# surftemp/cae_tools

Hardware: AMD Instinct MI355X
Metric: train images/sec (16x16->256x256, batch 64) (higher is better)
Workload: dtype f32

## Files before the change

cae_tools_amd/csrc/engine_choose.h:

```cpp
#pragma once

namespace {


#define S2_SHAPES(X) X(2, 1) X(4, 2) X(8, 4) X(6, 3)
#define S2_KERNELS(X, CI, CO) X(CI, CO, 3, 3) X(CI, CO, 4, 4) X(CI, CO, 3, 4) X(CI, CO, 4, 3)

template <int CI, int CO, int KH, int KW>
struct S2Shape { static constexpr int cin = CI, cout = CO, kh = KH, kw = KW; };

template <class F>
auto s2_for_shape(const ConvLayer& L, F fn) {
#define ONE(CI, CO, KH_, KW_) \
    if (L.cin == CI && L.cout == CO && L.kh == KH_ && L.kw == KW_) return fn(S2Shape<CI, CO, KH_, KW_>{});
#define PAIR(CI, CO) S2_KERNELS(ONE, CI, CO)
    S2_SHAPES(PAIR)
#undef PAIR
#undef ONE
    return false;
}

bool s2_shape_ok(const ConvLayer& L) { return L.transposed && L.stride == 2 && s2_for_shape(L, [](auto) { return true; }); }

bool s2_eligible(const cae_engine* e, const ConvLayer& L) { return e->use_s2 && L.sh_w >= 0 && s2_shape_ok(L); }
// ... 308 lines not shown
        if (h.n_seg + 1 > kHeadMaxSeg) return no("segments");
        h.o_bias[i] = take(cnt);
        h.seg[h.n_seg++] = HeadSeg{e->params + e->fc[i].b_off, i == 3 ? std::min(cnt, e->fc[3].nout) : cnt, h.o_bias[i], i == 3 ? 1 : 0};
    }
    for (int i = 0; i < 4; i++) {
        if (e->fc[i].nin % 4) return no("nin4");
        const int tiles = i == 3 ? h.tiles_per_wg : (e->fc[i].nout + 15) / 16;
        h.fc_split[i] = stage_split(tiles, e->fc[i].nin);
    }
    lds_bytes = (size_t)align_up(top, 4) * sizeof(float);
    return lds_bytes <= 152 * 1024 || no("lds");
}


bool tail_plan(const cae_engine* e, const StepArgs& a, TailArgs& t, size_t& lds_bytes, const char** why = nullptr) {
    auto no = [&](const char* reason) {
        if (why) *why = reason;
        return false;
    };
    if (!e->use_s2) return no("mode");
    if (a.syncing()) return no("syncing");
    if (e->variational) return no("variational");
    memset(&t, 0, sizeof t);
    const ConvLayer& P = e->enc.back();
    double* acc = e->gradacc();
    t.B = a.batch;
    for (int i = 0; i < 3; i++) {
        const FcLayer& F = e->fc[i];
        if (F.nin % 4 || F.nout % 4) return no("fc4");
        if (16 * F.nout / 4 > 2 * kHeadThreads) return no("panel");
        HeadFc& f = t.fc[i];
        f.nin = F.nin; f.nout = F.nout; f.relu = F.relu ? 1 : 0;
        f.w = e->params + F.w_off; f.bias = e->params + F.b_off;
        f.act = e->fptr(F.act_off); f.grad = e->fptr(F.grad_off);
        f.w_acc = acc + F.w_off; f.b_acc = acc + F.b_off;
        t.w4[i] = F.nin * F.nout / 4;
        if (t.w4[i] > 2 * kHeadThreads) return no("weights");
        const int r16 = (F.nin + 15) / 16 * 16;
        t.ldw[i] = r16 % 32 == 0 ? r16 + 16 : r16;
    }
    if (P.cout > kHeadMaxC || e->fc[0].nin != P.cout * P.hout * P.wout) return no("channels");
    t.y_last = e->fptr(P.act_off);
    t.g_last = e->fptr(P.grad_off);
    t.gamma = e->params + P.gamma_off;
    t.beta = e->params + P.beta_off;
    t.saved = e->bn_saved(P.bn_index);
    t.stats = e->bn_stats(P.bn_index);
    t.C = P.cout;
    t.hw = P.hout * P.wout;
    auto ld_of = [](int n) { return (n + 31) / 32 * 32 + 4; };
    t.ld2 = ld_of(e->fc[2].nout);
    t.ld1 = ld_of(e->fc[1].nout);
    t.ld0 = ld_of(e->fc[0].nout);
    int64_t top = 0;
    auto take = [&](int64_t floats) { return lds_take(top, floats); };
    t.o_c = take(4 * (int64_t)P.cout);
    t.o_red = take(2 * 2 * (int64_t)kHeadWaves);
    t.o_g2 = take(16 * (int64_t)t.ld2 + 32);
    t.o_g1 = take(16 * (int64_t)t.ld1 + 32);
    t.o_g0 = take(16 * (int64_t)t.ld0 + 32);
    t.o_y = take(16 * (int64_t)e->fc[0].nin + 32);
    t.o_gx = take(16 * (int64_t)e->fc[0].nin + 32);
    top = align_up(top, 4);
    t.zero4 = (int)((top - t.o_g2) / 4);
    int64_t wmax = 0;
    for (int i = 0; i < 3; i++) wmax = std::max<int64_t>(wmax, (int64_t)e->fc[i].nout * t.ldw[i]);
    t.o_w = take(wmax + 64);
    t.o_part = take(kHeadWaves * 256);
    lds_bytes = (size_t)align_up(top, 4) * sizeof(float);
    if (lds_bytes > 152 * 1024) return no("lds");
    for (int i = 0; i < 3; i++) t.sp_d[i] = stage_split((e->fc[2 - i].nin + 15) / 16, e->fc[2 - i].nout);
    for (int i = 0; i < 3; i++) t.sp_w[i] = stage_split(((e->fc[2 - i].nout + 15) / 16) * ((e->fc[2 - i].nin + 16) / 16), 16);
    return true;
}

enum DecFwdK {
    DF_FUSED_LAST,
    DF_ROWS,
    DF_S2,
    DF_CT_LDS,
    DF_IG,
    DF_UP
};
enum DecBwdK {
    DB_FUSED_LAST,
    DB_ROWS,
    DB_S2,
    DB_CT_LDS,
    DB_IG,
    DB_GENERIC
};

int s2_fwd_epi(const cae_engine* e, int l, bool train, bool external_loss) {
    if (l + 1 < (int)e->dec.size()) return train ? S2_RAW_STATS : S2_RAW;
    if (external_loss) return S2_RAW;
    return train ? S2_SIGMSE : S2_SIGOUT;
}

bool rows_ok(const cae_engine* e, const ConvLayer& L, int l) {
    return l + 1 < (int)e->dec.size() && l > 0 && e->dec[l - 1].has_bn && rows_bwd_ok(e, L);
}

DecFwdK choose_dec_fwd(const cae_engine* e, const ConvLayer& L, int l, int B, bool train, bool external_loss) {
    const bool last = l + 1 == (int)e->dec.size();
    if (last && train && !external_loss && last_fused_ok(e, L)) return DF_FUSED_LAST;
    if (rows_ok(e, L, l)) return DF_ROWS;
    if (s2_eligible(e, L)) return DF_S2;
    if (e->use_s2 && !last && L.stride == 2 && L.kh <= 4 && L.kw <= 4) {
        CtFwd c;
        int waves = 0;
        size_t lds = 0;
        return ct_fwd_plan(e, B, L, l, c, waves, lds) ? DF_CT_LDS : DF_IG;
    }
    return DF_UP;
}

DecBwdK choose_dec_bwd(const cae_engine* e, const ConvLayer& L, int l, int B, bool external_loss) {
    const bool last = l + 1 == (int)e->dec.size();
    if (last && !external_loss && last_fused_ok(e, L)) return DB_FUSED_LAST;
    if (rows_ok(e, L, l)) return DB_ROWS;
    if (s2_eligible(e, L)) return DB_S2;
    if (e->use_s2) {
        CtBwdPlan p;
        return ct_bwd_plan(e, B, L, l, p) ? DB_CT_LDS : DB_IG;
    }
    return DB_GENERIC;
}

bool enc_conv0_fits_adam(const cae_engine* e, const StepArgs& a, const ConvLayer& L) {
    return e->use_s2 && !a.syncing() && a.world == 1 && L.cout <= 64 &&
           (int64_t)L.cin * L.cout * L.kh * L.kw <= 4096 && (int64_t)a.batch * L.hout * L.wout < kDivSmallMaxN &&
           L.hout * L.wout < kDivSmallMaxD && L.in_elems() < (1 << 24) && L.out_elems() < (1 << 24) &&
           (int64_t)a.batch * L.in_elems() < (1 << 30) && (int64_t)a.batch * L.out_elems() < (1 << 30) &&
           e->bn_stat_off[L.bn_index] == e->off_zero_begin;
}

bool enc_conv0_in_adam_ok(const cae_engine* e, const StepArgs& a, const ConvLayer& L) {
    return a.adam_follows && e->x_published && enc_conv0_fits_adam(e, a, L);
}

const char* head_staging(const HeadArgs& h) {
    const int per = h.enc[0].cin * h.enc[0].hin * h.enc[0].win;
    if (per & 3) return "scalar";
    return h.B * (per >> 2) <= 4 * kHeadThreads ? "direct" : "gather4";
}

}

extern "C" {

int cae_debug_plan(const cae_engine* e, int batch, int train, char* out, int64_t out_bytes) {
    if (!e || !out || out_bytes < 1) return fail(CAE_ERR_ARG, "cae_debug_plan: bad argument");
    if (batch < 1 || batch > e->max_batch) return fail(CAE_ERR_ARG, "cae_debug_plan: batch %d outside 1 .. %d", batch, e->max_batch);
    const bool tr = train != 0, ext = e->variational;
    const StepArgs a{0, nullptr, batch, batch, batch, tr, true, nullptr, nullptr, false};
    std::string s;
    char line[512];
    bool head_fused = false;
    {
        HeadArgs h;
        size_t lds = 0;
        const char* why = "";
        head_fused = head_plan(e, a, h, lds, &why);
        if (head_fused) {
            int straddle = 0;
            for (int j = 0; j < kHeadW4 && j * kHeadThreads < h.w_total4; j++) straddle += h.piece_m[j] == -1;
            const int T = (e->fc[3].nout + 15) / 16;
            snprintf(line, sizeof line,
                     "head fwd=fused enc=%d grid=%dx%d stage=%s w4=%d late=%d straddle=%d fc0=%d:%d fc1=%d:%d fc2=%d:%d fc3=%d:%d lds=%zu\n",
                     h.n_enc, (batch + 15) / 16, (T + h.tiles_per_wg - 1) / h.tiles_per_wg, head_staging(h), h.w_total4,
                     (int)(h.w_total4 > kHeadEarly * kHeadThreads), straddle, h.fc_split[0].lg, h.fc_split[0].per, h.fc_split[1].lg,
                     h.fc_split[1].per, h.fc_split[2].lg, h.fc_split[2].per, h.fc_split[3].lg, h.fc_split[3].per, lds);
        } else {
            snprintf(line, sizeof line, "head fwd=layers why=%s\n", why);
        }
        s += line;
    }
    static const char* const kEpiName[] = {"raw_stats", "sigmse", "sigout", "raw"};
    for (int l = 0; l < (int)e->dec.size(); l++) {
        const ConvLayer& L = e->dec[l];
        const int ci = L.cin, co = L.cout, kh = L.kh, kw = L.kw;
        char f[128], b[256];
        switch (choose_dec_fwd(e, L, l, batch, tr, ext)) {
            case DF_FUSED_LAST: {
                const LastPick p = choose_last(L, l > 0 && e->dec[l - 1].has_bn);
                snprintf(f, sizeof f, "last_fused<%d,%d,%d,%d> hb=%d vec4=%d bn=%d", ci, co, kh, kw, kLastHB, (int)p.vec4, (int)p.bn);
                break;
            }
            case DF_ROWS: {
                const RowsPick p = choose_rows_fwd(L);
                snprintf(f, sizeof f, "s2_fwd_rows<%d,%d,%d,%d>", ci, co, p.hb, 64 / p.lw);
                break;
            }
            case DF_S2: {
                const int epi = s2_fwd_epi(e, l, tr, ext);
                const S2FwdPick p = choose_s2_fwd(L, batch, epi);
                const char* fam = p.k == S2F_CS ? "s2_fwd_cs" : (p.k == S2F_QUAD ? "s2_fwd" : "s2_fwd2");
                snprintf(f, sizeof f, "%s<%d,%d,%d,%d,%d> epi=%s", fam, ci, co, kh, kw, p.tw, kEpiName[epi]);
                break;
            }
            case DF_CT_LDS: snprintf(f, sizeof f, "ct_fwd_lds<%d,%d>", kh, kw); break;
            case DF_IG: snprintf(f, sizeof f, "ig_fwd_s2"); break;
            case DF_UP: snprintf(f, sizeof f, "up"); break;
        }
        if (!tr) {
            snprintf(b, sizeof b, "-");
        } else {
            switch (choose_dec_bwd(e, L, l, batch, ext)) {
                case DB_FUSED_LAST: snprintf(b, sizeof b, "(fused)"); break;
                case DB_ROWS: {
                    const RowsPick p = choose_rows_bwd(L);
                    snprintf(b, sizeof b, "s2_bwd_rows<%d,%d,%d,3,3,%d,%d,%d>", ci, ci == 4 ? 4 : 2, co, p.hb, 64 / p.lw, p.d);
                    break;
                }
                case DB_S2: {
                    const S2BwdPick p = choose_s2_bwd(L);
                    if (p.k == S2B_DIRECT) snprintf(b, sizeof b, "s2_bwd2<%d,%d,%d,%d,%d>", ci, co, kh, kw, p.tw);
                    else if (p.k == S2B_SPLIT) snprintf(b, sizeof b, "s2_bwd_split<%d,%d,%d,%d,%d,%d>", ci, p.ct, co, kh, kw, p.tw);
                    else snprintf(b, sizeof b, "s2_bwd<%d,%d,%d,%d,%d>", ci, p.ct, co, kh, kw);
                    break;
                }
                case DB_CT_LDS: {
                    CtBwdPlan p;
                    (void)ct_bwd_plan(e, batch, L, l, p);
                    snprintf(b, sizeof b, "ct_bwd_lds ctb_kernel=%s ctb_imgs=%d ctb_groups=%d ctb_parts=%d ctb_bands=%d ctb_hb=%d ctb_sharded=%d",
                             p.bands > 1 ? "band" : "lds", p.imgs, p.groups, p.parts, p.bands, p.hb, (int)(L.sh_w >= 0));
                    break;
                }
                case DB_IG: {
                    const IgBwdPlan p = ig_bwd_plan(L, batch);
                    snprintf(b, sizeof b, "ig_bwd_pair ig_ksplit=%d ig_tpw=%d ig_chunks=%d ig_per=%d ig_dgroup=%d ig_wn8=%d", p.ksplit,
                             p.tiles_per_wave, p.chunks, p.per, p.d_group, p.w_n8);
                    break;
                }
                case DB_GENERIC: snprintf(b, sizeof b, "wgrad+down"); break;
            }
        }
        snprintf(line, sizeof line, "dec%d fwd=%s bwd=%s\n", l, f, b);
        s += line;
    }
    {
        TailArgs t;
        size_t lds = 0;
        const char* why = "";
        if (!tr) {
            snprintf(line, sizeof line, "tail bwd=-\n");
        } else if (tail_plan(e, a, t, lds, &why)) {
            const int rows = (batch + 15) / 16;
            snprintf(line, sizeof line, "tail bwd=fused rows=%d sums=%s g1=%d:%d g0=%d:%d gx=%d:%d w2=%d:%d w1=%d:%d w0=%d:%d lds=%zu\n", rows,
                     rows <= kStatShards ? "stored" : "added", t.sp_d[0].lg, t.sp_d[0].per, t.sp_d[1].lg, t.sp_d[1].per, t.sp_d[2].lg,
                     t.sp_d[2].per, t.sp_w[0].lg, t.sp_w[0].per, t.sp_w[1].lg, t.sp_w[1].per, t.sp_w[2].lg, t.sp_w[2].per, lds);
        } else {
            snprintf(line, sizeof line, "tail bwd=layers why=%s\n", why);
        }
        s += line;
    }
    if (tr) {
        const bool in_adam = head_fused && enc_conv0_fits_adam(e, a, e->enc[0]);
        snprintf(line, sizeof line, "enc conv0=%s inner=%s\n", in_adam ? "adam" : "own",
                 e->enc.size() < 2 ? "-" : (e->use_s2 && !a.syncing() ? "pair" : "layers"));
        s += line;
    }
    if ((int64_t)s.size() + 1 > out_bytes)
        return fail(CAE_ERR_ARG, "cae_debug_plan: the report needs %zu bytes, got %lld", s.size() + 1, (long long)out_bytes);
    memcpy(out, s.c_str(), s.size() + 1);
    return CAE_OK;
}

}
```

cae_tools_amd/csrc/kernels_last.h:

```cpp
#pragma once
#include <utility>
#include "kernels_s2.h"

namespace cae {

template <class F, int... Is>
__device__ __forceinline__ void static_for_impl(F&& f, std::integer_sequence<int, Is...>) {
    (f(std::integral_constant<int, Is>{}), ...);
}
template <int N, class F>
__device__ __forceinline__ void static_for(F&& f) {
    static_for_impl(f, std::make_integer_sequence<int, N>{});
}

struct S2Last {
    int B, H, W, OH, OW;
    int QH, QW;
    int strips, bands;
    int total;
    const float* in;
    BnDesc bn_in;
    const float* w;
    const float* bias;
    const float* target;
    const int* perm;
    int use_cursor;
    const StepState* st;
    double* losses;
    float inv_count;
    double* bias_acc;
    double* wacc;
    int acc_stride;
    float* gin;
    double* stats_in;
};

constexpr int kLastStripPx = 127;

__device__ __forceinline__ float uniform_f(float v) {
    return __builtin_bit_cast(float, __builtin_amdgcn_readfirstlane(__builtin_bit_cast(int, v)));
}
__device__ __forceinline__ float from_left(float v, float edge) {
    return __builtin_bit_cast(float, __builtin_amdgcn_update_dpp(__builtin_bit_cast(int, edge), __builtin_bit_cast(int, v), 0x138, 0xF, 0xF, false));
}
__device__ __forceinline__ float from_right(float v, float edge) {
    return __builtin_bit_cast(float, __builtin_amdgcn_update_dpp(__builtin_bit_cast(int, edge), __builtin_bit_cast(int, v), 0x130, 0xF, 0xF, false));
}

constexpr int kWsumLd = 68;
constexpr int kWsumScratch = 16 * kWsumLd;
template <int N>
__device__ __forceinline__ void wave_sums_lds(const float (&v)[N], float* scr, float* out, int lane) {
    const int row = lane >> 2, qd = lane & 3;
#pragma unroll
    for (int c0 = 0; c0 < N; c0 += 16) {
#pragma unroll
        for (int i = 0; i < 16; i++)
            if (c0 + i < N) scr[i * kWsumLd + lane] = v[c0 + i];
        const float4* p = reinterpret_cast<const float4*>(scr + row * kWsumLd + 4 * qd);
        const float4 a0 = p[0], a1 = p[4], a2 = p[8], a3 = p[12];
        float t = ((a0.x + a0.y) + (a0.z + a0.w)) + ((a1.x + a1.y) + (a1.z + a1.w)) + ((a2.x + a2.y) + (a2.z + a2.w)) +
                  ((a3.x + a3.y) + (a3.z + a3.w));
        t += dpp_f<0xB1>(t);
        t += dpp_f<0x4E>(t);
        if (qd == 0 && c0 + row < N) out[c0 + row] = t;
    }
}

template <int CIN, int COUT, int KH, int KW, int HB, bool VEC4, bool BN>
__global__ void __launch_bounds__(256) __attribute__((amdgpu_waves_per_eu(1, 2))) k_s2_last_fused(S2Last a) {
    kernarg_warm<sizeof(S2Last)>();
    constexpr int NACC = CIN * COUT * KH * KW;
    constexpr int NRED = NACC + 2 * CIN;
    constexpr int NR = HB + 1;
    static_assert(KH >= 3 && KH <= 4 && KW >= 3 && KW <= 4, "3- or 4-tap stride-2 kernels");
    __shared__ float redf[4 * NRED];
    __shared__ double redd[4 * 2 * COUT];
    __shared__ __attribute__((aligned(16))) float wscr[4 * kWsumScratch];
    __shared__ float xch[4 * CIN * 2 * 64];

    const int tid = threadIdx.x, lane = tid & 63;
    const int wv = __builtin_amdgcn_readfirstlane(tid >> 6);
    const unsigned HW = a.H * a.W, OHW = a.OH * a.OW;

    const int item = blockIdx.x * 4 + wv;
    const bool work = item < a.total;
    const int it = work ? item : 0;
    const int b = it / (a.strips * a.bands);
    const int rem = it - b * (a.strips * a.bands);
    const int band = rem / a.strips, strip = rem - band * a.strips;
    const int m0 = band * HB;
    const bool last_band = band == a.bands - 1, last_strip = strip == a.strips - 1;
    const int n0 = strip * kLastStripPx + 2 * lane;
    const bool multi = a.strips > 1;
    const bool has_below = !multi && work && wv < 3 && band + 1 < a.bands;
    const int nrows = has_below ? HB : NR;
    const bool all_cols = VEC4 && 256 <= a.OW;

    int lane_zero = 0;
    asm volatile("" : "+v"(lane_zero));
    long long bs_v = 0;
    const bool indirect = a.perm != nullptr || a.use_cursor != 0;
    if (indirect) bs_v = (&a.st->batch_start)[lane_zero];
    const int loss_slot_v = (&a.st->loss_slot)[lane_zero];
    double sa = 0.0, sb = 0.0;
    float gam[CIN], bet[CIN], rmn[CIN], rvr[CIN];
    if constexpr (BN) {
        static_assert(CIN <= 8, "one lane per (channel, shard)");
        if (lane < 8 * CIN) {
            const double2 t = *reinterpret_cast<const double2*>(a.bn_in.stats + ((size_t)(lane & 7) * CIN + (lane >> 3)) * 4);
            sa = t.x;
            sb = t.y;
        }
#pragma unroll
        for (int ci = 0; ci < CIN; ci++) {
            gam[ci] = a.bn_in.gamma[ci];
            bet[ci] = a.bn_in.beta[ci];
            rmn[ci] = a.bn_in.rmean[ci];
            rvr[ci] = a.bn_in.rvar[ci];
        }
    }
    float wk[NACC], bk[COUT];
#pragma unroll
    for (int i = 0; i < NACC; i++) wk[i] = a.w[i];
#pragma unroll
    for (int i = 0; i < COUT; i++) bk[i] = a.bias[i];
    asm volatile("" ::: "memory");
    __builtin_amdgcn_sched_barrier(0);
    int perm_val_v;
    if (a.perm) perm_val_v = a.perm[bs_v + b + lane_zero];
    constexpr int NLEFT = VEC4 ? 1 : NR + 1;
    float rin[NR + 1][CIN][2], rleft[NLEFT][CIN];
    float4 tgt[NR][COUT][2];
    {
        const float* inb = a.in + (size_t)b * CIN * HW;
        const int c0 = min(n0, a.W - 1), c1 = min(n0 + 1, a.W - 1), cl = min(max(n0 - 1, 0), a.W - 1);
#pragma unroll
        for (int r = 0; r <= NR; r++) {
            const unsigned ro = (unsigned)min(max(m0 - 1 + r, 0), a.H - 1) * a.W;
#pragma unroll
            for (int ci = 0; ci < CIN; ci++) {
                rin[r][ci][0] = inb[ci * HW + ro + c0];
                rin[r][ci][1] = inb[ci * HW + ro + c1];
                if constexpr (!VEC4) {
                    rleft[r][ci] = 0.f;
                    if (multi && lane == 0) rleft[r][ci] = inb[ci * HW + ro + cl];
                }
            }
        }
        asm volatile("" ::: "memory");
        __builtin_amdgcn_sched_barrier(0);
        const long long bs = ((long long)__builtin_amdgcn_readfirstlane((int)(bs_v >> 32)) << 32) |
                             (unsigned)__builtin_amdgcn_readfirstlane((int)bs_v);
        const long long tb = a.perm ? (long long)__builtin_amdgcn_readfirstlane(perm_val_v) : bs + b;
#pragma unroll
        for (int r = 0; r < NR; r++) {
            if (r >= nrows) break;
#pragma unroll
            for (int co = 0; co < COUT; co++) {
                const float* plane = a.target + ((size_t)tb * COUT + co) * (size_t)OHW;
#pragma unroll
                for (int py = 0; py < 2; py++) {
                    const unsigned ro = (unsigned)min(2 * (m0 + r) + py, a.OH - 1) * a.OW;
                    const int ox = 2 * n0;
                    if constexpr (VEC4) {
                        tgt[r][co][py] = *reinterpret_cast<const float4*>(plane + ro + min(ox, a.OW - 4));
                    } else {
                        tgt[r][co][py].x = plane[ro + min(ox, a.OW - 1)];
                        tgt[r][co][py].y = plane[ro + min(ox + 1, a.OW - 1)];
                        tgt[r][co][py].z = plane[ro + min(ox + 2, a.OW - 1)];
                        tgt[r][co][py].w = plane[ro + min(ox + 3, a.OW - 1)];
                    }
                }
            }
        }
        asm volatile("" ::: "memory");
        __builtin_amdgcn_sched_barrier(0);
    }
#pragma unroll
    for (int i = 0; i < NACC; i++) wk[i] = uniform_f(wk[i]);
#pragma unroll
    for (int i = 0; i < COUT; i++) bk[i] = uniform_f(bk[i]);
    float4 kc[CIN];
#pragma unroll
    for (int ci = 0; ci < CIN; ci++) kc[ci] = make_float4(0.f, 1.f, 0.f, 1.f);
    if constexpr (BN) {
        sa += dpp_d<0xB1>(sa); sb += dpp_d<0xB1>(sb);
        sa += dpp_d<0x4E>(sa); sb += dpp_d<0x4E>(sb);
        sa += dpp_d<0x141>(sa); sb += dpp_d<0x141>(sb);
        const long long ba = __builtin_bit_cast(long long, sa), bb = __builtin_bit_cast(long long, sb);
#pragma unroll
        for (int ci = 0; ci < CIN; ci++) {
            const int lo1 = __builtin_amdgcn_readlane((int)ba, 8 * ci), hi1 = __builtin_amdgcn_readlane((int)(ba >> 32), 8 * ci);
            const int lo2 = __builtin_amdgcn_readlane((int)bb, 8 * ci), hi2 = __builtin_amdgcn_readlane((int)(bb >> 32), 8 * ci);
            const double s1 = __builtin_bit_cast(double, ((long long)hi1 << 32) | (unsigned)lo1);
            const double s2 = __builtin_bit_cast(double, ((long long)hi2 << 32) | (unsigned)lo2);
            const double mu = s1 * a.bn_in.inv_count;
            double var = s2 * a.bn_in.inv_count - mu * mu;
            var = var < 0.0 ? 0.0 : var;
            const float mean = (float)mu;
            const float invstd = 1.0f / sqrtf((float)(var + (double)a.bn_in.eps));
            kc[ci] = make_float4(mean, uniform_f(gam[ci]) * invstd, uniform_f(bet[ci]), invstd);
            if (blockIdx.x == 0 && tid == 0 && a.bn_in.update) {
                a.bn_in.saved[2 * ci] = mean;
                a.bn_in.saved[2 * ci + 1] = invstd;
                a.bn_in.rmean[ci] = (1.f - a.bn_in.momentum) * rmn[ci] + a.bn_in.momentum * mean;
                a.bn_in.rvar[ci] = (1.f - a.bn_in.momentum) * rvr[ci] + a.bn_in.momentum * (float)(var * a.bn_in.unbias);
            }
        }
    }

    float dw[NACC];
#pragma unroll
    for (int i = 0; i < NACC; i++) dw[i] = 0.f;
    float d1[CIN], d2[CIN];
#pragma unroll
    for (int i = 0; i < CIN; i++) d1[i] = d2[i] = 0.f;
    float ls[COUT], gs[COUT];
#pragma unroll
    for (int i = 0; i < COUT; i++) ls[i] = gs[i] = 0.f;

    auto activate = [&](int r, int ci, float (&act)[3]) {
        const int y = m0 - 1 + r;
        const bool rowok = y >= 0 && y < a.H;
        float v0 = rin[r][ci][0], v1 = rin[r][ci][1], vl = VEC4 ? 0.f : rleft[VEC4 ? 0 : r][ci];
        if constexpr (BN) {
            v0 = fmaxf(0.f, fmaf(v0 - kc[ci].x, kc[ci].y, kc[ci].z));
            v1 = fmaxf(0.f, fmaf(v1 - kc[ci].x, kc[ci].y, kc[ci].z));
            vl = fmaxf(0.f, fmaf(vl - kc[ci].x, kc[ci].y, kc[ci].z));
        }
        act[1] = (rowok && n0 < a.W) ? v0 : 0.f;
        act[2] = (rowok && n0 + 1 < a.W) ? v1 : 0.f;
        const float edge = (!VEC4 && rowok && n0 >= 1) ? vl : 0.f;
        act[0] = from_left(act[2], edge);
    };

    float actP[CIN][3];
    float carry[CIN][2];
#pragma unroll
    for (int ci = 0; ci < CIN; ci++) {
        activate(0, ci, actP[ci]);
        carry[ci][0] = carry[ci][1] = 0.f;
    }

    float xsave[CIN][2];
#pragma unroll
    for (int ci = 0; ci < CIN; ci++) xsave[ci][0] = xsave[ci][1] = 0.f;
    {
        static_for<NR>([&](auto R) {
            constexpr int r = decltype(R)::value;
            const int m = m0 + r;
            if (work && r < nrows && m < a.QH) {
            const bool own_row = r < HB || last_band;
            float actN[CIN][3];
#pragma unroll
            for (int ci = 0; ci < CIN; ci++) activate(r + 1, ci, actN[ci]);

            float g[COUT][2][2][2];
#pragma unroll
            for (int co = 0; co < COUT; co++) {
                float acc[2][2][2];
#pragma unroll
                for (int q = 0; q < 2; q++)
#pragma unroll
                    for (int py = 0; py < 2; py++)
#pragma unroll
                        for (int px = 0; px < 2; px++) acc[q][py][px] = bk[co];
#pragma unroll
                for (int ci = 0; ci < CIN; ci++) {
                    const float* wc = &wk[(ci * COUT + co) * KH * KW];
#pragma unroll
                    for (int q = 0; q < 2; q++)
#pragma unroll
                        for (int j = 0; j < 2; j++)
#pragma unroll
                            for (int i = 0; i < 2; i++) {
                                const float av = j ? actP[ci][1 + q - i] : actN[ci][1 + q - i];
#pragma unroll
                                for (int py = 0; py < 2; py++)
#pragma unroll
                                    for (int px = 0; px < 2; px++)
                                        if (py + 2 * j < KH && px + 2 * i < KW)
                                            acc[q][py][px] = fmaf(av, wc[(py + 2 * j) * KW + px + 2 * i], acc[q][py][px]);
                            }
                }
#pragma unroll
                for (int py = 0; py < 2; py++) {
                    const float tv[4] = {tgt[r][co][py].x, tgt[r][co][py].y, tgt[r][co][py].z, tgt[r][co][py].w};
                    const bool rowok = 2 * m + py < a.OH;
#pragma unroll
                    for (int q = 0; q < 2; q++)
#pragma unroll
                        for (int px = 0; px < 2; px++) {
                            const int ox = 2 * (n0 + q) + px;
                            const bool valid = rowok && (all_cols || ox < a.OW);
                            const float yh = sigmoid_fast(acc[q][py][px]);
                            const float d = valid ? yh - tv[2 * q + px] : 0.f;
                            const float gv = (2.0f * d * a.inv_count) * (yh * (1.0f - yh));
                            g[co][q][py][px] = gv;
                            if constexpr (VEC4) {
                                if (own_row) { ls[co] = fmaf(d, d, ls[co]); gs[co] += gv; }
                            } else {
                                const bool own = own_row && (q == 0 || lane < 63 || last_strip);
                                const float dl = own ? d : 0.f;
                                ls[co] = fmaf(dl, dl, ls[co]);
                                gs[co] += own ? gv : 0.f;
                            }
                        }
                }
            }
            float P[CIN][2][2][2];
#pragma unroll
            for (int ci = 0; ci < CIN; ci++) {
#pragma unroll
                for (int q = 0; q < 2; q++)
#pragma unroll
                    for (int j = 0; j < 2; j++)
#pragma unroll
                        for (int i = 0; i < 2; i++) P[ci][q][j][i] = 0.f;
#pragma unroll
                for (int co = 0; co < COUT; co++) {
                    const float* wc = &wk[(ci * COUT + co) * KH * KW];
#pragma unroll
                    for (int q = 0; q < 2; q++) {
                        const bool ownq = VEC4 || q == 0 || lane < 63 || last_strip;
#pragma unroll
                        for (int j = 0; j < 2; j++)
#pragma unroll
                            for (int i = 0; i < 2; i++) {
                                const float av = j ? actP[ci][1 + q - i] : actN[ci][1 + q - i];
                                const float avw = ownq ? av : 0.f;
#pragma unroll
                                for (int py = 0; py < 2; py++)
#pragma unroll
                                    for (int px = 0; px < 2; px++)
                                        if (py + 2 * j < KH && px + 2 * i < KW) {
                                            const int t = (py + 2 * j) * KW + px + 2 * i;
                                            P[ci][q][j][i] = fmaf(g[co][q][py][px], wc[t], P[ci][q][j][i]);
                                            if (own_row) dw[(ci * COUT + co) * KH * KW + t] = fmaf(avw, g[co][q][py][px], dw[(ci * COUT + co) * KH * KW + t]);
                                        }
                            }
                    }
                }
            }
            const int y = m - 1;
            const bool emit = r >= 1 && y < a.H;
            float tj1[CIN][2], tj0[CIN][2];
#pragma unroll
            for (int ci = 0; ci < CIN; ci++) {
                tj1[ci][0] = P[ci][0][1][0] + P[ci][1][1][1];
                tj0[ci][0] = P[ci][0][0][0] + P[ci][1][0][1];
                tj1[ci][1] = P[ci][1][1][0] + from_right(P[ci][0][1][1], 0.f);
                tj0[ci][1] = P[ci][1][0][0] + from_right(P[ci][0][0][1], 0.f);
                if (r == 0) { xsave[ci][0] = tj1[ci][0]; xsave[ci][1] = tj1[ci][1]; }
            }
            if (emit) {
                const bool p0 = n0 < a.W, p1 = n0 + 1 < a.W && lane < 63;
#pragma unroll
                for (int ci = 0; ci < CIN; ci++) {
                    float gv0 = carry[ci][0] + tj1[ci][0], gv1 = carry[ci][1] + tj1[ci][1];
                    if constexpr (BN) {
                        const float e0 = rin[r][ci][0] - kc[ci].x, e1 = rin[r][ci][1] - kc[ci].x;
                        gv0 = fmaf(e0, kc[ci].y, kc[ci].z) > 0.f ? gv0 : 0.f;
                        gv1 = fmaf(e1, kc[ci].y, kc[ci].z) > 0.f ? gv1 : 0.f;
                        const float s0 = p0 ? gv0 : 0.f, s1 = p1 ? gv1 : 0.f;
                        d1[ci] += s0 + s1;
                        d2[ci] = fmaf(s0, e0 * kc[ci].w, fmaf(s1, e1 * kc[ci].w, d2[ci]));
                    }
                    float* gp = a.gin + (size_t)(b * CIN + ci) * HW + (unsigned)y * a.W + n0;
                    if (p0) {
                        gp[0] = gv0;
                        gp[p1 ? 1 : 0] = p1 ? gv1 : gv0;
                    }
                }
            }
#pragma unroll
            for (int ci = 0; ci < CIN; ci++) {
                carry[ci][0] = tj0[ci][0];
                carry[ci][1] = tj0[ci][1];
#pragma unroll
                for (int k = 0; k < 3; k++) actP[ci][k] = actN[ci][k];
            }
            }
            if constexpr (r == 0) {
#pragma unroll
                for (int ci = 0; ci < CIN; ci++) {
                    xch[((wv * CIN + ci) * 2 + 0) * 64 + lane] = xsave[ci][0];
                    xch[((wv * CIN + ci) * 2 + 1) * 64 + lane] = xsave[ci][1];
                }
                __syncthreads();
            }
        });
    }
    if (has_below) {
        const int y = m0 + HB - 1;
        if (y < a.H) {
            const bool p0 = n0 < a.W, p1 = n0 + 1 < a.W && lane < 63;
#pragma unroll
            for (int ci = 0; ci < CIN; ci++) {
                float gv0 = carry[ci][0] + xch[(((wv + 1) * CIN + ci) * 2 + 0) * 64 + lane];
                float gv1 = carry[ci][1] + xch[(((wv + 1) * CIN + ci) * 2 + 1) * 64 + lane];
                if constexpr (BN) {
                    const float e0 = rin[HB][ci][0] - kc[ci].x, e1 = rin[HB][ci][1] - kc[ci].x;
                    gv0 = fmaf(e0, kc[ci].y, kc[ci].z) > 0.f ? gv0 : 0.f;
                    gv1 = fmaf(e1, kc[ci].y, kc[ci].z) > 0.f ? gv1 : 0.f;
                    const float s0 = p0 ? gv0 : 0.f, s1 = p1 ? gv1 : 0.f;
                    d1[ci] += s0 + s1;
                    d2[ci] = fmaf(s0, e0 * kc[ci].w, fmaf(s1, e1 * kc[ci].w, d2[ci]));
                }
                float* gp = a.gin + (size_t)(b * CIN + ci) * HW + (unsigned)y * a.W + n0;
                if (p0) {
                    gp[0] = gv0;
                    gp[p1 ? 1 : 0] = p1 ? gv1 : gv0;
                }
            }
        }
    }

    {
        float red[NRED];
#pragma unroll
        for (int i = 0; i < NACC; i++) red[i] = dw[i];
#pragma unroll
        for (int c = 0; c < CIN; c++) {
            red[NACC + 2 * c] = d1[c];
            red[NACC + 2 * c + 1] = d2[c];
        }
        wave_sums_lds<NRED>(red, wscr + wv * kWsumScratch, redf + wv * NRED, lane);
    }
#pragma unroll
    for (int co = 0; co < COUT; co++) {
        const double t1 = wave_sum_lane63((double)ls[co] * (double)a.inv_count), t2 = wave_sum_lane63((double)gs[co]);
        if (lane == 63) {
            redd[(wv * COUT + co) * 2] = t1;
            redd[(wv * COUT + co) * 2 + 1] = t2;
        }
    }
    __syncthreads();
    const int shard = blockIdx.x & (kStatShards - 1);
    for (int j = tid; j < NRED + 2 * COUT; j += 256) {
        if (j < NRED) {
            const double s = (double)redf[j] + (double)redf[NRED + j] + (double)redf[2 * NRED + j] + (double)redf[3 * NRED + j];
            if (j < NACC) {
                acc_add<ACC_GRAD>(&a.wacc[(size_t)shard * a.acc_stride + j], s);
            } else if (a.stats_in) {
                const int jj = j - NACC;
                acc_add<ACC_GRAD>(&a.stats_in[((size_t)shard * CIN + (jj >> 1)) * 4 + 2 + (jj & 1)], s);
            }
        } else {
            const int q = j - NRED, co = q >> 1, which = q & 1;
            double s = 0.0;
#pragma unroll
            for (int w = 0; w < 4; w++) s += redd[(w * COUT + co) * 2 + which];
            if (which == 0) acc_add<ACC_GRAD>(&a.losses[(size_t)loss_slot_v * kStatShards + shard], s);
            else acc_add<ACC_GRAD>(&a.bias_acc[(size_t)shard * a.acc_stride + co], s);
        }
    }
    asm volatile("" :: "v"(perm_val_v));
}

}
```

cae_tools_amd/csrc/kernels_rows.h:

```cpp
#pragma once
#include "kernels_last.h"

namespace cae {

struct S2Rows {
    int B, H, W, OH, OW;
    int QH;
    int bands;
    int groups;
    const float* g;
    const float* yout;
    BnDesc bn_out;
    const float* ain;
    BnDesc bn_in;
    const float* w;
    float* gin;
    double* stats_in;
    double* wacc;
    int wacc_stride;
    BnGradOut bg;
};

template <int CIN, int CT, int COUT, int KH, int KW, int HB, int IMGS, int D>
__global__ void __launch_bounds__(256) __attribute__((amdgpu_waves_per_eu(1, 2))) k_s2_bwd_rows(S2Rows a) {
    kernarg_warm<sizeof(S2Rows)>();
    constexpr int CS = CIN / CT;
    constexpr int NB = 4 / CS;
    constexpr int LW = 64 / IMGS;
    constexpr int NACC = CT * COUT * KH * KW;
    constexpr int NRED = NACC + 2 * CT;
    constexpr int NR = HB + 1;
    static_assert(CS * NB == 4 && CS * CT == CIN, "four waves");
    static_assert(KH == 3 && KW == 3, "3x3 stride-2 kernels");
    static_assert(CIN <= 8 && COUT <= 8, "one lane per (channel, shard) in the BatchNorm prologue");
    __shared__ float redf[4 * NRED];
    __shared__ __attribute__((aligned(16))) float wscr[4 * kWsumScratch];
    __shared__ float xch[NB > 1 ? 4 * CT * 64 : 1];
    __shared__ __attribute__((aligned(16))) float wl[CIN * COUT * 12];

    const int tid = threadIdx.x, lane = tid & 63;
    const int wv = __builtin_amdgcn_readfirstlane(tid >> 6);
    const int cgrp = wv % CS, bsel = wv / CS;
    const int c0 = cgrp * CT;
    const int sub = lane / LW, n = lane - sub * LW;
    const unsigned HW = a.H * a.W, OHW = a.OH * a.OW;

    const int wg_bands = (a.bands + NB - 1) / NB;
    const int grp = blockIdx.x / wg_bands, bg0 = blockIdx.x - grp * wg_bands;
    const int band = bg0 * NB + bsel;
    const bool band_ok = band < a.bands;
    const int m0 = band * HB;
    const int b = grp * IMGS + sub;
    const bool img_ok = b < a.B;
    const int bc = img_ok ? b : a.B - 1;
    const bool has_below = NB > 1 && bsel + 1 < NB && band + 1 < a.bands;
    const int nrows = has_below ? HB : NR;

    float4 ko[COUT], ki[CT];
    double sa = 0.0, sb = 0.0;
    if (lane < 8 * COUT) {
        const double2 t = *reinterpret_cast<const double2*>(a.bn_out.stats + ((size_t)(lane & 7) * COUT + (lane >> 3)) * 4 + 2);
        sa = t.x;
        sb = t.y;
    }
    float mean_o[COUT], istd_o[COUT], gam_o[COUT];
#pragma unroll
    for (int co = 0; co < COUT; co++) {
        mean_o[co] = a.bn_out.saved[2 * co];
        istd_o[co] = a.bn_out.saved[2 * co + 1];
        gam_o[co] = a.bn_out.gamma[co];
    }
    float mean_i[CT], istd_i[CT], gam_i[CT], bet_i[CT];
#pragma unroll
    for (int c = 0; c < CT; c++) {
        mean_i[c] = a.bn_in.saved[2 * (c0 + c)];
        istd_i[c] = a.bn_in.saved[2 * (c0 + c) + 1];
        gam_i[c] = a.bn_in.gamma[c0 + c];
        bet_i[c] = a.bn_in.beta[c0 + c];
    }
    constexpr int NWL = (CIN * COUT * 12 + 255) / 256;
    float wreg[NWL];
#pragma unroll
    for (int u = 0; u < NWL; u++) {
        const int i = min(tid + 256 * u, CIN * COUT * 12 - 1), cc = i / 12, t = i - cc * 12;
        wreg[u] = a.w[cc * 9 + min(t, 8)];
    }
    asm volatile("" ::: "memory");
    __builtin_amdgcn_sched_barrier(0);

    float2 rg[NR][COUT][2], ry[NR][COUT][2];
    float rin[NR + 1][CT];
    const float* gb = a.g + (size_t)bc * COUT * OHW;
    const float* yb = a.yout + (size_t)bc * COUT * OHW;
    const float* ib = a.ain + ((size_t)bc * CIN + c0) * HW;
    const bool pair_ok = 2 * n + 1 < a.OW;
    const int oxc = pair_ok ? 2 * n : min(max(2 * n - 1, 0), a.OW - 2);
    const int xc = min(n, a.W - 1);
    const bool last_band = band == a.bands - 1;
    auto load_in = [&](auto R) {
        constexpr int r = decltype(R)::value;
        const unsigned ro = (unsigned)min(max(m0 - 1 + r, 0), a.H - 1) * a.W;
#pragma unroll
        for (int c = 0; c < CT; c++) rin[r][c] = ib[c * HW + ro + xc];
    };
    auto load_g = [&](auto R) {
        constexpr int r = decltype(R)::value;
        if (r >= nrows) return;
#pragma unroll
        for (int co = 0; co < COUT; co++)
#pragma unroll
            for (int py = 0; py < 2; py++) {
                const unsigned off = co * OHW + (unsigned)min(2 * (m0 + r) + py, a.OH - 1) * a.OW + oxc;
                rg[r][co][py] = *reinterpret_cast<const float2*>(gb + off);
                ry[r][co][py] = *reinterpret_cast<const float2*>(yb + off);
            }
    };
    load_in(std::integral_constant<int, 0>{});
    static_for<(D < NR ? D : NR)>([&](auto R) {
        constexpr int r = decltype(R)::value;
        load_in(std::integral_constant<int, r + 1>{});
        load_g(R);
    });
    __builtin_amdgcn_sched_barrier(0);
    {
        sa += dpp_d<0xB1>(sa); sb += dpp_d<0xB1>(sb);
        sa += dpp_d<0x4E>(sa); sb += dpp_d<0x4E>(sb);
        sa += dpp_d<0x141>(sa); sb += dpp_d<0x141>(sb);
        const long long ba = __builtin_bit_cast(long long, sa), bb = __builtin_bit_cast(long long, sb);
#pragma unroll
        for (int co = 0; co < COUT; co++) {
            const int lo1 = __builtin_amdgcn_readlane((int)ba, 8 * co), hi1 = __builtin_amdgcn_readlane((int)(ba >> 32), 8 * co);
            const int lo2 = __builtin_amdgcn_readlane((int)bb, 8 * co), hi2 = __builtin_amdgcn_readlane((int)(bb >> 32), 8 * co);
            const double dbeta = __builtin_bit_cast(double, ((long long)hi1 << 32) | (unsigned)lo1);
            const double dgamma = __builtin_bit_cast(double, ((long long)hi2 << 32) | (unsigned)lo2);
            const float mean = uniform_f(mean_o[co]), invstd = uniform_f(istd_o[co]);
            const float scale = uniform_f(gam_o[co]) * invstd;
            ko[co] = make_float4(mean, scale, (float)((double)scale * dbeta * a.bn_out.inv_count),
                                 (float)((double)scale * (double)invstd * dgamma * a.bn_out.inv_count));
            if (blockIdx.x == 0 && tid == 0 && a.bg.stats) {
                a.bg.beta_acc[co] = dbeta * a.bg.scale;
                a.bg.gamma_acc[co] = dgamma * a.bg.scale;
            }
        }
#pragma unroll
        for (int c = 0; c < CT; c++) {
            const float invstd = uniform_f(istd_i[c]);
            ki[c] = make_float4(uniform_f(mean_i[c]), uniform_f(gam_i[c]) * invstd, uniform_f(bet_i[c]), invstd);
        }
#pragma unroll
        for (int u = 0; u < NWL; u++) {
            const int i = tid + 256 * u;
            if (i < CIN * COUT * 12) wl[i] = (i % 12) < 9 ? wreg[u] : 0.f;
        }
    }
// ... 143 lines not shown
    }
    __syncthreads();
    const int shard = blockIdx.x & (kStatShards - 1);
    for (int i = tid; i < CS * NRED; i += 256) {
        const int gsel = i / NRED, j = i - gsel * NRED;
        double s = 0.0;
#pragma unroll
        for (int q = 0; q < NB; q++) s += (double)redf[(q * CS + gsel) * NRED + j];
        if (j < NACC) {
            acc_add<ACC_GRAD>(&a.wacc[(size_t)shard * a.wacc_stride + (size_t)gsel * NACC + j], s);
        } else {
            const int jj = j - NACC;
            acc_add<ACC_GRAD>(&a.stats_in[((size_t)shard * CIN + gsel * CT + (jj >> 1)) * 4 + 2 + (jj & 1)], s);
        }
    }
}

}

namespace cae {

struct S2FwdRows {
    int B, H, W, OH, OW;
    int QH;
    int bands, groups;
    const float* in;
    BnDesc bn_in;
    const float* w;
    const float* bias;
    float* out;
    double* stats;
};

template <int CIN, int COUT, int HB, int IMGS>
__global__ void __launch_bounds__(256) k_s2_fwd_rows(S2FwdRows a) {
    kernarg_warm<sizeof(S2FwdRows)>();
    constexpr int KH = 3, KW = 3;
    constexpr int LW = 64 / IMGS;
    constexpr int NRED = 2 * COUT;
    static_assert(CIN <= 8, "one lane per (channel, shard) in the BatchNorm prologue");
    __shared__ float redf[4 * NRED];
    __shared__ __attribute__((aligned(16))) float wscr[4 * kWsumScratch];
    __shared__ __attribute__((aligned(16))) float wl[CIN * COUT * 12];

    const int tid = threadIdx.x, lane = tid & 63;
    const int wv = __builtin_amdgcn_readfirstlane(tid >> 6);
    const int sub = lane / LW, n = lane - sub * LW;
    const unsigned HW = a.H * a.W, OHW = a.OH * a.OW;
    const int wg_bands = (a.bands + 3) / 4;
    const int grp = blockIdx.x / wg_bands, bg0 = blockIdx.x - grp * wg_bands;
    const int band = bg0 * 4 + wv;
    const bool band_ok = band < a.bands;
    const int m0 = band * HB;
    const int b = grp * IMGS + sub;
    const bool img_ok = b < a.B;
    const int bc = img_ok ? b : a.B - 1;

    float4 ki[CIN];
    const bool batch = a.bn_in.mode == BN_BATCH;
    double sa = 0.0, sb = 0.0;
    if (batch && lane < 8 * CIN) {
        const double2 t = *reinterpret_cast<const double2*>(a.bn_in.stats + ((size_t)(lane & 7) * CIN + (lane >> 3)) * 4);
        sa = t.x;
        sb = t.y;
    }
    float gam[CIN], bet[CIN], rmn[CIN], rvr[CIN];
#pragma unroll
    for (int c = 0; c < CIN; c++) {
        gam[c] = a.bn_in.gamma[c];
        bet[c] = a.bn_in.beta[c];
        rmn[c] = a.bn_in.rmean[c];
        rvr[c] = a.bn_in.rvar[c];
    }
    constexpr int NWL = (CIN * COUT * 12 + 255) / 256;
    float wreg[NWL];
#pragma unroll
    for (int u = 0; u < NWL; u++) {
        const int i = min(tid + 256 * u, CIN * COUT * 12 - 1), cc = i / 12, t = i - cc * 12;
        wreg[u] = a.w[cc * 9 + min(t, 8)];
    }
    float bk[COUT];
#pragma unroll
    for (int co = 0; co < COUT; co++) bk[co] = a.bias[co];
    asm volatile("" ::: "memory");
    __builtin_amdgcn_sched_barrier(0);

    float rin[HB + 1][CIN];
    {
        const float* ib = a.in + (size_t)bc * CIN * HW;
        const int xc = min(n, a.W - 1);
#pragma unroll
        for (int r = 0; r <= HB; r++) {
            const unsigned ro = (unsigned)min(max(m0 - 1 + r, 0), a.H - 1) * a.W;
#pragma unroll
            for (int c = 0; c < CIN; c++) rin[r][c] = ib[c * HW + ro + xc];
        }
    }
    __builtin_amdgcn_sched_barrier(0);
    {
        sa += dpp_d<0xB1>(sa); sb += dpp_d<0xB1>(sb);
        sa += dpp_d<0x4E>(sa); sb += dpp_d<0x4E>(sb);
        sa += dpp_d<0x141>(sa); sb += dpp_d<0x141>(sb);
        const long long ba = __builtin_bit_cast(long long, sa), bb = __builtin_bit_cast(long long, sb);
#pragma unroll
        for (int c = 0; c < CIN; c++) {
            float mean, invstd;
            if (batch) {
                const int lo1 = __builtin_amdgcn_readlane((int)ba, 8 * c), hi1 = __builtin_amdgcn_readlane((int)(ba >> 32), 8 * c);
                const int lo2 = __builtin_amdgcn_readlane((int)bb, 8 * c), hi2 = __builtin_amdgcn_readlane((int)(bb >> 32), 8 * c);
                const double s1 = __builtin_bit_cast(double, ((long long)hi1 << 32) | (unsigned)lo1);
                const double s2 = __builtin_bit_cast(double, ((long long)hi2 << 32) | (unsigned)lo2);
                const double mu = s1 * a.bn_in.inv_count;
                double var = s2 * a.bn_in.inv_count - mu * mu;
                var = var < 0.0 ? 0.0 : var;
                mean = (float)mu;
                invstd = 1.0f / sqrtf((float)(var + (double)a.bn_in.eps));
                if (blockIdx.x == 0 && tid == 0 && a.bn_in.update) {
                    a.bn_in.saved[2 * c] = mean;
                    a.bn_in.saved[2 * c + 1] = invstd;
                    a.bn_in.rmean[c] = (1.f - a.bn_in.momentum) * rmn[c] + a.bn_in.momentum * mean;
                    a.bn_in.rvar[c] = (1.f - a.bn_in.momentum) * rvr[c] + a.bn_in.momentum * (float)(var * a.bn_in.unbias);
                }
            } else {
                mean = uniform_f(rmn[c]);
                invstd = 1.0f / sqrtf(uniform_f(rvr[c]) + a.bn_in.eps);
            }
            ki[c] = make_float4(mean, uniform_f(gam[c]) * invstd, uniform_f(bet[c]), invstd);
        }
#pragma unroll
        for (int u = 0; u < NWL; u++) {
            const int i = tid + 256 * u;
            if (i < CIN * COUT * 12) wl[i] = (i % 12) < 9 ? wreg[u] : 0.f;
        }
#pragma unroll
        for (int co = 0; co < COUT; co++) bk[co] = uniform_f(bk[co]);
    }
    __syncthreads();

    auto activate = [&](int r, int c, float (&act)[2]) {
        const int y = m0 - 1 + r;
        const float v = fmaxf(0.f, fmaf(rin[r][c] - ki[c].x, ki[c].y, ki[c].z));
        act[1] = (y >= 0 && y < a.H && n < a.W) ? v : 0.f;
        const float left = from_left(act[1], 0.f);
        act[0] = n == 0 ? 0.f : left;
    };
    float actP[CIN][2];
#pragma unroll
    for (int c = 0; c < CIN; c++) activate(0, c, actP[c]);
    float s1[COUT], s2[COUT];
#pragma unroll
    for (int co = 0; co < COUT; co++) s1[co] = s2[co] = 0.f;
    const bool pair_ok = 2 * n + 1 < a.OW;
    float* ob = a.out + (size_t)bc * COUT * OHW;

    static_for<HB>([&](auto R) {
        constexpr int r = decltype(R)::value;
        const int m = m0 + r;
        if (m < a.QH && band_ok) {
            float actN[CIN][2];
#pragma unroll
            for (int c = 0; c < CIN; c++) activate(r + 1, c, actN[c]);
            int wofs = 0;
            asm volatile("" : "+v"(wofs));
#pragma unroll
            for (int co = 0; co < COUT; co++) {
                float acc[2][2] = {{bk[co], bk[co]}, {bk[co], bk[co]}};
#pragma unroll
                for (int c = 0; c < CIN; c++) {
                    float wc[12];
                    {
                        const float4* wq = reinterpret_cast<const float4*>(&wl[(c * COUT + co) * 12 + wofs]);
                        const float4 w0 = wq[0], w1 = wq[1], w2 = wq[2];
                        wc[0] = w0.x; wc[1] = w0.y; wc[2] = w0.z; wc[3] = w0.w; wc[4] = w1.x; wc[5] = w1.y; wc[6] = w1.z; wc[7] = w1.w;
                        wc[8] = w2.x; wc[9] = w2.y; wc[10] = w2.z; wc[11] = w2.w;
                    }
#pragma unroll
                    for (int j = 0; j < 2; j++)
#pragma unroll
                        for (int i = 0; i < 2; i++) {
                            const float av = j ? actP[c][1 - i] : actN[c][1 - i];
#pragma unroll
                            for (int py = 0; py < 2; py++)
#pragma unroll
                                for (int px = 0; px < 2; px++)
                                    if (py + 2 * j < KH && px + 2 * i < KW)
                                        acc[py][px] = fmaf(av, wc[(py + 2 * j) * KW + px + 2 * i], acc[py][px]);
                        }
                }
#pragma unroll
                for (int py = 0; py < 2; py++) {
                    const int oy = 2 * m + py;
                    const bool ok0 = img_ok && oy < a.OH && 2 * n < a.OW, ok1 = ok0 && pair_ok;
                    float* op = ob + co * OHW + (unsigned)min(oy, a.OH - 1) * a.OW + min(2 * n, a.OW - 1);
                    if (ok1) *reinterpret_cast<float2*>(op) = make_float2(acc[py][0], acc[py][1]);
                    else if (ok0) op[0] = acc[py][0];
                    const float v0 = ok0 ? acc[py][0] : 0.f, v1 = ok1 ? acc[py][1] : 0.f;
                    s1[co] += v0 + v1;
                    s2[co] = fmaf(v0, v0, fmaf(v1, v1, s2[co]));
                }
            }
#pragma unroll
            for (int c = 0; c < CIN; c++) {
                actP[c][0] = actN[c][0];
                actP[c][1] = actN[c][1];
            }
        }
    });
    if (!a.stats) return;
    {
        float red[NRED];
#pragma unroll
        for (int co = 0; co < COUT; co++) {
            red[2 * co] = s1[co];
            red[2 * co + 1] = s2[co];
        }
        wave_sums_lds<NRED>(red, wscr + wv * kWsumScratch, redf + wv * NRED, lane);
    }
    __syncthreads();
    if (tid < NRED) {
        const double s = (double)redf[tid] + (double)redf[NRED + tid] + (double)redf[2 * NRED + tid] + (double)redf[3 * NRED + tid];
        acc_add<ACC_STAT>(&a.stats[((size_t)(blockIdx.x & (kStatShards - 1)) * COUT + (tid >> 1)) * 4 + (tid & 1)], s);
    }
}

}
```

cae_tools_amd/engine.py:

```python
import ctypes as C
from collections import OrderedDict

import numpy as np
import torch

from . import _lib
from ._engine_base import TEST, TRAIN, SpecPlan, _spec_layers, _to_c, require_gpu
from ._lib import CaeError, check


class EnginePlan(SpecPlan):

    PREFIX = "cae_"

    def bn_prefixes(self):
        return [n[: -len(".running_mean")] for n in self.tensors if n.endswith(".running_mean")]

    def set_kernel_mode(self, mode):
        check(self.lib.cae_set_kernel_mode(self.handle, int(mode)))

    def kernel_plan(self, batch, train):
        buf = C.create_string_buffer(1 << 16)
        check(self.lib.cae_debug_plan(self.handle, int(batch), 1 if train else 0, buf, len(buf)))
        plan = {}
        for line in buf.value.decode().splitlines():
            (name, *fields) = line.split()
            plan[name] = dict(f.split("=", 1) for f in fields)
        return plan


class HipEngine(EnginePlan):

    def __init__(self, spec, fc_size, latent_size, max_batch, device=None, graph=True, specialised=True):
        require_gpu()
        super().__init__(spec, fc_size, latent_size, max_batch)
        self._bind(device, grads=True, buffers=True)
        check(self.lib.cae_set_graph_mode(self.handle, 1 if graph else 0))
        check(self.lib.cae_set_kernel_mode(self.handle, int(specialised) if isinstance(specialised, int) and not isinstance(specialised, bool) else (1 if specialised else 0)))
        torch.cuda.synchronize(self.device)
        self.num_batches_tracked = 0
        self.adam_steps = 0
        self._datasets = {}
        self._keep = []
        self.loss_slots = int(self.lib.cae_loss_slots(self.handle))
        self._slot = 0
        self._cursor = None

    def grad_view(self, name):
        (arena, off, numel, shape) = self.tensors[name]
        assert arena == 0
        return self.grads[off:off + numel].view(shape)

    def export_state(self):
        (enc, dec) = super().export_state()
        return self._ordered(enc), self._ordered(dec)

    @staticmethod
    def _ordered(sd):
        order = {"weight": 0, "bias": 1, "running_mean": 2, "running_var": 3, "num_batches_tracked": 4}
        groups = OrderedDict()
        for k in sd:
            groups.setdefault(k.rsplit(".", 1)[0], []).append(k)
        out = OrderedDict()
        for g, keys in groups.items():
            for k in sorted(keys, key=lambda s: order[s.rsplit(".", 1)[1]]):
                out[k] = sd[k]
        return out

    def reset_optimizer(self):
        self.sync()
        self.exp_avg.zero_()
        self.exp_avg_sq.zero_()
        self.adam_steps = 0
        torch.cuda.synchronize(self.device)
        check(self.lib.cae_set_adam_step(self.handle, 0))

    def load_optimizer_state(self, moments, step):
        self.sync()
        for name, (m, v) in moments.items():
            (arena, off, numel, shape) = self.tensors[name]
            self.exp_avg[off:off + numel].copy_(torch.as_tensor(m, dtype=torch.float32).reshape(-1).to(self.device))
            self.exp_avg_sq[off:off + numel].copy_(torch.as_tensor(v, dtype=torch.float32).reshape(-1).to(self.device))
        torch.cuda.synchronize(self.device)
        self.adam_steps = int(step)
        check(self.lib.cae_set_adam_step(self.handle, int(step)))

    def set_hyper(self, lr=1e-3, betas=(0.9, 0.999), eps=1e-8, weight_decay=1e-5):
        check(self.lib.cae_set_hyper(self.handle, float(lr), float(betas[0]), float(betas[1]), float(eps),
                                     float(weight_decay)))

    def set_lr(self, lr):
        check(self.lib.cae_set_lr(self.handle, float(lr)))

    def _same_device(self, a, what):
        if a.device != self.device:
            raise CaeError(f"{what} lives on {a.device} but this engine runs on {self.device} "
                           "(select the rank's GPU before creating data sets: cae_tools_amd.dp.select_device)")

    def set_dataset(self, which, x, t=None):
        for name, a, shp in (("x", x, self.in_shape), ("t", t, self.out_shape)):
            if a is None:
                continue
            if a.dtype != torch.float32 or not a.is_cuda or not a.is_contiguous():
                raise CaeError(f"dataset {name} must be a contiguous fp32 CUDA tensor")
            self._same_device(a, f"dataset {name}")
            if tuple(a.shape[1:]) != tuple(shp):
                raise CaeError(f"dataset {name} has sample shape {tuple(a.shape[1:])}, model expects {tuple(shp)}")
        self.sync()
        torch.cuda.synchronize(self.device)
        self._datasets[which] = (x, t)
        check(self.lib.cae_set_dataset(self.handle, which, x.data_ptr(), t.data_ptr() if t is not None else None,
                                       int(x.shape[0])))

    def upload_perm(self, perm):
        p = torch.as_tensor(np.asarray(perm, dtype=np.int32)).to(self.device)
        torch.cuda.synchronize(self.device)
        self._keep.append(p)
        if len(self._keep) > 64:
            self.sync()
            self._keep = self._keep[-8:]
        return p

    def _claim_slots(self, n):
        if n > self.loss_slots:
            raise CaeError(f"{n} steps between loss reads exceeds {self.loss_slots} slots")
        if self._slot + n > self.loss_slots:
            self._slot = 0
        first = self._slot
        self._slot += n
        return first

    def _set_cursor(self, start, slot):
        if self._cursor != (int(start), int(slot)):
            check(self.lib.cae_set_cursor(self.handle, int(start), int(slot)))
        self._cursor = (int(start), int(slot))

    def _advance(self, samples, steps):
        if self._cursor is not None:
            self._cursor = (self._cursor[0] + int(samples), self._cursor[1] + int(steps))

    def _read_losses(self, first, n):
        out = (C.c_double * n)()
        check(self.lib.cae_read_losses(self.handle, first, n, out))
        return [float(v) for v in out]

    def run_batches(self, which, perm_dev, n, batch_size, train=True):
        nb = (n + batch_size - 1) // batch_size
        first = self._claim_slots(nb)
        ptr = perm_dev.data_ptr() if perm_dev is not None else None
        self._set_cursor(0, first)
        self._enqueue(which, ptr, n, batch_size, train)
        self._advance(n, nb)
        if train:
            self.num_batches_tracked += nb
            self.adam_steps += nb
        return self._read_losses(first, nb)

    STEPS_PER_GRAPH = 64

    def _enqueue(self, which, ptr, n, batch_size, train):
        many = self.lib.cae_train_steps if train else self.lib.cae_eval_steps
        one = self.lib.cae_train_step if train else self.lib.cae_eval_step
        full = n // batch_size
        while full >= self.STEPS_PER_GRAPH:
            check(many(self.handle, which, ptr, batch_size, self.STEPS_PER_GRAPH))
            full -= self.STEPS_PER_GRAPH
        if full > 1:
            check(many(self.handle, which, ptr, batch_size, full))
        elif full == 1:
            check(one(self.handle, which, ptr, batch_size))
        if n % batch_size:
            check(one(self.handle, which, ptr, n % batch_size))

    def capture_graphs(self):
        import contextlib

# ... 217 lines not shown
```

Baseline: 391,800.

## Stage decoder output and grad-input rows in LDS and flush as aligned 16-byte stores

The rows forward kernel and the fused-last backward kernel now write their per-lane output pixels into a per-wave LDS slab. Each wave then flushes whole row runs with aligned 16-byte global stores using the sc1 cache bit, plus scalar stores for the unaligned head and tail. This replaces scattered float2 and scalar global writes, aiming for fuller memory transactions on the large 256x256 activations. It adds LDS traffic, inline assembly with an s_nop, and extra index arithmetic. The debug plan can now report which store path each layer uses.

```diff
diff --git a/cae_tools_amd/csrc/engine_choose.h b/cae_tools_amd/csrc/engine_choose.h
--- a/cae_tools_amd/csrc/engine_choose.h
+++ b/cae_tools_amd/csrc/engine_choose.h
@@ -484,7 +484,7 @@
 int cae_debug_plan(const cae_engine* e, int batch, int train, char* out, int64_t out_bytes) {
     if (!e || !out || out_bytes < 1) return fail(CAE_ERR_ARG, "cae_debug_plan: bad argument");
     if (batch < 1 || batch > e->max_batch) return fail(CAE_ERR_ARG, "cae_debug_plan: batch %d outside 1 .. %d", batch, e->max_batch);
-    const bool tr = train != 0, ext = e->variational;
+    const bool tr = (train & 1) != 0, with_stores = (train & 2) != 0, ext = e->variational;
     const StepArgs a{0, nullptr, batch, batch, batch, tr, true, nullptr, nullptr, false};
     std::string s;
     char line[512];
@@ -513,6 +513,8 @@
         const ConvLayer& L = e->dec[l];
         const int ci = L.cin, co = L.cout, kh = L.kh, kw = L.kw;
         char f[128], b[256];
+        const bool f_run16 = choose_dec_fwd(e, L, l, batch, tr, ext) == DF_ROWS;
+        const bool b_run16 = tr && choose_dec_bwd(e, L, l, batch, ext) == DB_FUSED_LAST;
         switch (choose_dec_fwd(e, L, l, batch, tr, ext)) {
             case DF_FUSED_LAST: {
                 const LastPick p = choose_last(L, l > 0 && e->dec[l - 1].has_bn);
@@ -568,8 +570,15 @@
                 case DB_GENERIC: snprintf(b, sizeof b, "wgrad+down"); break;
             }
         }
-        snprintf(line, sizeof line, "dec%d fwd=%s bwd=%s\n", l, f, b);
-        s += line;
+        if (with_stores) {
+            snprintf(line, sizeof line, "dec%d fwd=%s fwd.stores=%s bwd=%s", l, f, f_run16 ? "run16" : "plain", b);
+            s += line;
+            if (tr) s += b_run16 ? " bwd.stores=run16" : " bwd.stores=plain";
+            s += "\n";
+        } else {
+            snprintf(line, sizeof line, "dec%d fwd=%s bwd=%s\n", l, f, b);
+            s += line;
+        }
     }
     {
         TailArgs t;
diff --git a/cae_tools_amd/csrc/kernels_last.h b/cae_tools_amd/csrc/kernels_last.h
--- a/cae_tools_amd/csrc/kernels_last.h
+++ b/cae_tools_amd/csrc/kernels_last.h
@@ -1,6 +1,7 @@
 #pragma once
 #include <utility>
 #include "kernels_s2.h"
+#include "run_store.h"
 
 namespace cae {
 
@@ -243,6 +244,24 @@
         carry[ci][0] = carry[ci][1] = 0.f;
     }
 
+    static_assert(CIN % 2 == 0 && kWsumScratch / 2 >= kLastStripPx + 4 && (kWsumScratch / 2) % 4 == 0, "two channels' rows per flush");
+    float* const gslab = wscr + wv * kWsumScratch;
+    float* const gbase = a.gin + (size_t)b * CIN * HW;
+    const int gcol0 = strip * kLastStripPx;
+    const int gseg = min(kLastStripPx, a.W - gcol0);
+    const int gphase = run_phase(gbase);
+    auto gin_put = [&](int ci, int y, bool p0, bool p1, float gv0, float gv1) {
+        const int ph = (gphase + ci * HW + (unsigned)y * a.W + gcol0) & 3;
+        float* sp = gslab + (ci & 1) * (kWsumScratch / 2) + ph + 2 * lane;
+        if (p0) sp[0] = gv0;
+        if (p1) sp[1] = gv1;
+    };
+    auto gin_flush = [&](int ce, int y) {
+        const int half = lane >> 5;
+        const unsigned e = (ce + half) * HW + (unsigned)y * a.W + gcol0;
+        run_flush<32>(gslab + half * (kWsumScratch / 2), gbase + e, (gphase + e) & 3, gseg, lane & 31, true);
+    };
+
     float xsave[CIN][2];
 #pragma unroll
     for (int ci = 0; ci < CIN; ci++) xsave[ci][0] = xsave[ci][1] = 0.f;
@@ -367,11 +386,8 @@
                         d1[ci] += s0 + s1;
                         d2[ci] = fmaf(s0, e0 * kc[ci].w, fmaf(s1, e1 * kc[ci].w, d2[ci]));
                     }
-                    float* gp = a.gin + (size_t)(b * CIN + ci) * HW + (unsigned)y * a.W + n0;
-                    if (p0) {
-                        gp[0] = gv0;
-                        gp[p1 ? 1 : 0] = p1 ? gv1 : gv0;
-                    }
+                    gin_put(ci, y, p0, p1, gv0, gv1);
+                    if (ci & 1) gin_flush(ci - 1, y);
                 }
             }
 #pragma unroll
@@ -408,11 +424,8 @@
                     d1[ci] += s0 + s1;
                     d2[ci] = fmaf(s0, e0 * kc[ci].w, fmaf(s1, e1 * kc[ci].w, d2[ci]));
                 }
-                float* gp = a.gin + (size_t)(b * CIN + ci) * HW + (unsigned)y * a.W + n0;
-                if (p0) {
-                    gp[0] = gv0;
-                    gp[p1 ? 1 : 0] = p1 ? gv1 : gv0;
-                }
+                gin_put(ci, y, p0, p1, gv0, gv1);
+                if (ci & 1) gin_flush(ci - 1, y);
             }
         }
     }
diff --git a/cae_tools_amd/csrc/kernels_rows.h b/cae_tools_amd/csrc/kernels_rows.h
--- a/cae_tools_amd/csrc/kernels_rows.h
+++ b/cae_tools_amd/csrc/kernels_rows.h
@@ -1,5 +1,6 @@
 #pragma once
 #include "kernels_last.h"
+#include "run_store.h"
 
 namespace cae {
 
@@ -449,6 +450,8 @@
     for (int co = 0; co < COUT; co++) s1[co] = s2[co] = 0.f;
     const bool pair_ok = 2 * n + 1 < a.OW;
     float* ob = a.out + (size_t)bc * COUT * OHW;
+    static_assert(kWsumScratch / IMGS >= 4 * LW + 4 && (kWsumScratch / IMGS) % 4 == 0, "a row pair of 2 LW pixels per row + the phase");
+    float* slab = wscr + wv * kWsumScratch + sub * (kWsumScratch / IMGS);
 
     static_for<HB>([&](auto R) {
         constexpr int r = decltype(R)::value;
@@ -484,17 +487,20 @@
                                         acc[py][px] = fmaf(av, wc[(py + 2 * j) * KW + px + 2 * i], acc[py][px]);
                         }
                 }
+                float* rp = ob + co * OHW + (unsigned)(2 * m) * a.OW;
+                const int ph = run_phase(rp);
 #pragma unroll
                 for (int py = 0; py < 2; py++) {
                     const int oy = 2 * m + py;
                     const bool ok0 = img_ok && oy < a.OH && 2 * n < a.OW, ok1 = ok0 && pair_ok;
-                    float* op = ob + co * OHW + (unsigned)min(oy, a.OH - 1) * a.OW + min(2 * n, a.OW - 1);
-                    if (ok1) *reinterpret_cast<float2*>(op) = make_float2(acc[py][0], acc[py][1]);
-                    else if (ok0) op[0] = acc[py][0];
+                    float* sp = slab + ph + py * a.OW + 2 * n;
+                    if (ok0) sp[0] = acc[py][0];
+                    if (ok1) sp[1] = acc[py][1];
                     const float v0 = ok0 ? acc[py][0] : 0.f, v1 = ok1 ? acc[py][1] : 0.f;
                     s1[co] += v0 + v1;
                     s2[co] = fmaf(v0, v0, fmaf(v1, v1, s2[co]));
                 }
+                run_flush<LW>(slab, rp, ph, min(2, a.OH - 2 * m) * a.OW, n, img_ok);
             }
 #pragma unroll
             for (int c = 0; c < CIN; c++) {
diff --git a/cae_tools_amd/csrc/run_store.h b/cae_tools_amd/csrc/run_store.h
--- /dev/null
+++ b/cae_tools_amd/csrc/run_store.h
@@ -0,0 +1,28 @@
+#pragma once
+
+namespace cae {
+
+typedef float run_v4f __attribute__((ext_vector_type(4)));
+
+__device__ __forceinline__ void store16_wt(float* p, run_v4f v) {
+    asm volatile("global_store_dwordx4 %0, %1, off sc1\n\ts_nop 1" : : "v"(p), "v"(v) : "memory");
+}
+__device__ __forceinline__ void store4_wt(float* p, float v) {
+    __hip_atomic_store(p, v, __ATOMIC_RELAXED, __HIP_MEMORY_SCOPE_AGENT);
+}
+
+__device__ __forceinline__ int run_phase(const float* dst) { return (int)((reinterpret_cast<unsigned long long>(dst) >> 2) & 3); }
+
+template <int LW>
+__device__ __forceinline__ void run_flush(const float* slab, float* dst, int ph, int len, int n, bool on) {
+    const int end = ph + len;
+    const int k0 = (ph + 3) >> 2, k1 = max(end >> 2, k0);
+    float* g = dst - ph;
+    if (!on) return;
+    for (int k = k0 + n; k < k1; k += LW) store16_wt(g + 4 * k, *reinterpret_cast<const run_v4f*>(slab + 4 * k));
+    const int i = n < 4 ? ph + n : 4 * k1 + n - 4;
+    const bool ok = n < 4 ? (i < 4 * k0 && i < end) : (n < 8 && i < end);
+    if (ok) store4_wt(g + i, slab[i]);
+}
+
+}
diff --git a/cae_tools_amd/engine.py b/cae_tools_amd/engine.py
--- a/cae_tools_amd/engine.py
+++ b/cae_tools_amd/engine.py
@@ -19,9 +19,9 @@
     def set_kernel_mode(self, mode):
         check(self.lib.cae_set_kernel_mode(self.handle, int(mode)))
 
-    def kernel_plan(self, batch, train):
+    def kernel_plan(self, batch, train, stores=False):
         buf = C.create_string_buffer(1 << 16)
-        check(self.lib.cae_debug_plan(self.handle, int(batch), 1 if train else 0, buf, len(buf)))
+        check(self.lib.cae_debug_plan(self.handle, int(batch), (1 if train else 0) | (2 if stores else 0), buf, len(buf)))
         plan = {}
         for line in buf.value.decode().splitlines():
             (name, *fields) = line.split()
```

Result: no change. 394,800 (median of 6 runs) (+0.8%).
